# LI-Yiquan/3DPointCloudAttack

Measured on AMD Instinct MI355X. Metric: attack iters/s (B=32, N=1024, PointNet) + Chamfer HBM GB/s vs peak, higher is better.
Workload: dtype f32; 1 GPU; CW attack on PointNet(k=40, seeded random init), B=32 N=1024 fp32, UntargetedLogitsAdvLoss(kappa=30) + ChamferDist(adv2ori) + ClipPointsLinf(0.18), Adam lr 1e-2; one step = one hot-loop iteration for the whole batch; batch_per_gpu=32, points=1024, parallelism=independent attack instances x1

## Files before the change

3dpointcloudattack_amd/_lib.py:

```python
import ctypes
import os

import torch

from ctypes import c_char_p, c_float, c_int, c_int64, c_void_p

_HERE = os.path.dirname(os.path.abspath(__file__))
LIB_PATH = os.environ.get("PC3D_LIB_PATH") or os.path.join(_HERE, "libpc3d_hip.so")

_P = c_void_p
_I = c_int
_L = c_int64
_F = c_float
_D = ctypes.c_double
_PTS = [_P, _L, _L, _L]

SIGNATURES = {
    "pc3d_nn_f32": _PTS + _PTS + [_I, _I, _I, _P, _P, _P],
    "pc3d_nn_i64_f32": _PTS + _PTS + [_I, _I, _I, _P, _P, _P, _P],
    "pc3d_nn_bidir_f32": _PTS + _PTS + [_I, _I, _I, _P, _P, _P, _P, _P],
    "pc3d_nn_bidir_shared_ws_bytes": [_I, _I, _I],
    "pc3d_nn_bidir_shared_f32": _PTS + _PTS + [_I, _I, _I, _P, _P, _P, _P, _P, _L, _P],
    "pc3d_gemm_nt_f32": [_P, _L, _P, _P, _P, _L, _F, _I, _I, _I, _I, _F, _P, _L, _P],
    "pc3d_gemm_nt_tiled_f32": [_P, _L, _P, _P, _P, _L, _F, _I, _I, _I, _I, _F, _P, _L, _I, _P],
# ... 125 lines not shown
    "pc3d_pairwise_f32": _PTS + _PTS + [_I, _I, _I, _I, _P, _P],
    "pc3d_pointmlp3_tile_points": [],
    "pc3d_pointmlp3_max_fwd_f32": _PTS + [_I, _I] + [_P] * 7 + [_I, _I, _I, _I] + [_P] * 6 + [_P],
    "pc3d_pointmlp3_max_fwd_th_f32": _PTS + [_I, _I] + [_P, _P, _P, _I, _P] + [_P] * 6 + [_I, _I, _I, _I] + [_P] * 6 + [_P],
    "pc3d_pointmlp3_fold_f32": [_P, _P, _I, _I, _I, _I, _P, _P, _I, _P],
    "pc3d_pointmlp3_max_fwd_exact_f32": _PTS + [_I, _I] + [_P] * 7 + [_I, _I, _I, _I] + [_P] * 6 + [_P],
    "pc3d_pointmlp3_max_fwd_exact_th_f32": _PTS + [_I, _I] + [_P, _P, _P, _I, _P] + [_P] * 6 + [_I, _I, _I, _I] + [_P] * 6 + [_P],
    "pc3d_pointmlp3_max_fwd_screen_dbg_f32": _PTS + [_I, _I] + [_P, _P, _P, _P, _I, _P] + [_P] * 6 + [_I, _I, _I, _I]
    + [_P] * 6 + [_P, _P, _P, _I, _P],
    "pc3d_pointmlp3_w3_prepare_f32": [_P, _I, _P, _P, _P, _P],
    "pc3d_pointmlp3_max_fwd_prep_f32": _PTS + [_I, _I] + [_P] * 7 + [_I, _I, _I, _I] + [_P] * 6 + [_P, _P, _P] + [_P],
    "pc3d_pointmlp3_max_fwd_prep_th_f32": _PTS + [_I, _I] + [_P, _P, _P, _I, _P] + [_P] * 6 + [_I, _I, _I, _I] + [_P] * 6
    + [_P, _P, _P] + [_P],
    "pc3d_pointmlp3_max_fwd_screen_dbg_prep_f32": _PTS + [_I, _I] + [_P, _P, _P, _P, _I, _P] + [_P] * 6 + [_I, _I, _I, _I]
    + [_P] * 6 + [_P, _P, _P, _I] + [_P, _P, _P] + [_P],
    "pc3d_linear_pre_f32": [_P, _I, _I, _I, _P, _P, _I, _I, _I, _P, _I, _P, _I, _P, _I, _P],
    "pc3d_pointmlp3_max_bwd_f32": _PTS + [_I, _I] + [_P] * 7 + [_I, _I, _I] + [_P, _P, _P, _P] + _PTS + [_P, _I, _P],
    "pc3d_pointmlp3_max_bwd_twolist_f32": _PTS + [_I, _I] + [_P] * 7 + [_I, _I, _I] + [_P, _P, _P, _P] + _PTS + [_P, _I, _P],
    "pc3d_pointmlp3_max_bwd_tile32_f32": _PTS + [_I, _I] + [_P] * 7 + [_I, _I, _I] + [_P, _P, _P, _P] + _PTS + [_P, _I, _P],
    "pc3d_pointmlp3_max_bwd_packed_dbg_f32": _PTS + [_I, _I] + [_P] * 7 + [_I, _I, _I] + [_P, _P, _P, _P] + _PTS
    + [_P, _I, _I, _P],
    "pc3d_pointmlp3_bwd_tile_points": [],
    "pc3d_pointnet_ft_tower_fwd_f32": _PTS + [_I, _I] + [_P] * 6 + [_L] + [_P] * 3 + [_I] + [_P] * 5 + [_P],
    "pc3d_pointnet_ft_fold_w2_f32": [_P, _P, _I, _P, _P],
    "pc3d_pointnet_ft_tower_bwd_f32": _PTS + [_I, _I] + [_P] * 4 + [_L] + [_P, _P, _I] + [_P] * 5 + _PTS
    + [_P, _I, _I, _P, _I, _P],
    "pc3d_pointnet_ft_dtf_f32": _PTS + [_I, _I] + [_P] * 5 + [_P],
    "pc3d_linear_f32": [_P, _I, _I, _I, _I, _P, _P, _I, _I, _F, _P, _I, _F, _P, _I, _P],
    "pc3d_linear_nn_f32": [_P, _I, _I, _I, _I, _P, _P, _I, _I, _F, _P, _I, _F, _P, _I] + _PTS + _PTS
    + [_I, _I, _I, _P, _P, _I, _P],
# ... 77 lines not shown
```

3dpointcloudattack_amd/csrc/pointmlp.hip:

```cpp
#include <stdlib.h>
#include "pc3d_common.h"
#include "cw_update_body.h"
#include "pointmlp_body.h"

namespace pc3d {

__global__ __launch_bounds__(PM_FT) __attribute__((amdgpu_waves_per_eu(2, 2))) void pointmlp3_max_fwd_kernel(PMFwdArgs a) {
  __shared__ __attribute__((aligned(16))) float lds[PM_FWD_LDS_FLOATS];
  pm_fwd_prologue(a, lds);
  float* h2 = lds;
  const int tile = blockIdx.x, b = blockIdx.y;
  const int n0 = tile * PM_TP;
  const int lane = threadIdx.x & 63, wave = threadIdx.x >> 6;
  const int r = lane & 31, h = lane >> 5;

  const int ptile = wave & 3, cgrp = wave >> 2;
  float4 areg[PM_C2 / 8];
#pragma unroll
  for (int t = 0; t < PM_C2 / 8; ++t)
    areg[t] = *reinterpret_cast<const float4*>(h2 + (ptile * 32 + r) * PM_LD2 + 8 * t + 4 * h);
  __syncthreads();
  float* pv = lds;
  int* pi = reinterpret_cast<int*>(lds + 4 * PM_MAXC3F);
  const int nblk = a.C3 / 32;
// ... 1075 lines not shown
}

}

using namespace pc3d;

extern "C" int pc3d_pointmlp3_tile_points(void) { return PM_TP; }
extern "C" int pc3d_pointmlp3_bwd_tile_points(void) { return PM_BTP; }

static int pm_fwd_launch(const float* x, int64_t x_bs, int64_t x_ps, int64_t x_cs, int B, int N, const float* T,
                         const float* th_in, const float* th_W, const float* th_b, int th_K, float* th_out,
                         const float* W1, const float* b1, const float* W2, const float* b2, const float* W3,
                         const float* b3, int C1, int C2, int C3, int relu_last, float* part_val, int32_t* part_idx,
                         float* pooled, int32_t* argidx, uint64_t* mask1, uint32_t* mask2, void* stream,
                         bool exact = false, int32_t* stats = nullptr, float* dbg_S = nullptr, float* dbg_E = nullptr,
                         int stop_after = 0, const PMScreenPrep* prep = nullptr) {
  PC3D_REQUIRE(B >= 0 && N >= 1, "pc3d_pointmlp3_max_fwd_f32: bad sizes B=%d N=%d", B, N);
  PC3D_REQUIRE(C1 == PM_C1 && C2 == PM_C2 && C3 >= 32 && C3 % 32 == 0 && C3 <= PM_MAXC3F,
               "pc3d_pointmlp3_max_fwd_f32: unsupported widths %d/%d/%d (need 64/128/multiple of 32 <= 1024)", C1, C2, C3);
  PC3D_REQUIRE(B <= 65535, "pc3d_pointmlp3_max_fwd_f32: B=%d exceeds grid.y limit", B);
  if (B == 0) return PC3D_OK;
  PC3D_REQUIRE(x && W1 && b1 && W2 && b2 && W3 && b3 && part_val && part_idx,
               "pc3d_pointmlp3_max_fwd_f32: null pointer");
  PC3D_REQUIRE((pooled == nullptr) == (argidx == nullptr),
               "pc3d_pointmlp3_max_fwd_f32: pooled and argidx must both be given or both be NULL");
  PC3D_REQUIRE((mask1 == nullptr) == (mask2 == nullptr),
               "pc3d_pointmlp3_max_fwd_f32: mask1 and mask2 must both be given or both be NULL");
  const int ntiles = cdiv(N, PM_TP);
  PMFwdArgs a{{x, x_bs, x_ps, x_cs}, N, C3, ntiles, T, W1, b1, W2, b2, W3, b3, part_val, part_idx, mask1, mask2,
              th_in, th_W, th_b, th_K, th_out};
  hipStream_t st = as_stream(stream);
  int rc = 1;
  if (!exact) {
    rc = pm_fwd_screen_launch(a, B, stream, stats, dbg_S, dbg_E, stop_after, prep);
    if (rc < 0) return rc;
  }
  if (rc != 0) hipLaunchKernelGGL(pointmlp3_max_fwd_kernel, dim3(ntiles, B), dim3(PM_FT), 0, st, a);
  PC3D_LAUNCH_CHECK("pc3d_pointmlp3_max_fwd_f32");
  if (pooled) {
    hipLaunchKernelGGL(pointmlp3_fold_kernel<false>, dim3(cdiv(C3, 256), B), dim3(256), 0, st, part_val, part_idx, ntiles,
                       C3, relu_last, pooled, argidx);
    PC3D_LAUNCH_CHECK("pc3d_pointmlp3_max_fwd_f32/fold");
  }
  return PC3D_OK;
}

extern "C" int pc3d_pointmlp3_fold_f32(const float* part_val, const int32_t* part_idx, int B, int ntiles, int C3,
                                       int relu_last, float* pooled, int32_t* argidx, int serial, void* stream) {
  PC3D_REQUIRE(B >= 0 && B <= 65535 && ntiles >= 1 && C3 >= 1, "pc3d_pointmlp3_fold_f32: bad sizes B=%d ntiles=%d C3=%d", B,
// ... 122 lines not shown
                                                          const float* W3, const float* b3, int C1, int C2, int C3,
                                                          int relu_last, float* part_val, int32_t* part_idx, float* pooled,
                                                          int32_t* argidx, uint64_t* mask1, uint32_t* mask2, int32_t* stats,
                                                          float* dbg_S, float* dbg_E, int stop_after, const void* w3_bf,
                                                          const float* w3_nw, const float* w3_q, void* stream) {
  PC3D_REQUIRE(stats != nullptr, "pc3d_pointmlp3_max_fwd_screen_dbg_prep_f32: stats [B, ntiles, 2] is required");
  PC3D_REQUIRE((dbg_S == nullptr) == (dbg_E == nullptr), "pc3d_pointmlp3_max_fwd_screen_dbg_prep_f32: dbg_S and dbg_E go together");
  PC3D_REQUIRE(stop_after >= 0 && stop_after <= 3, "pc3d_pointmlp3_max_fwd_screen_dbg_prep_f32: stop_after = %d", stop_after);
  PC3D_REQUIRE(th_in == nullptr || (T == nullptr && th_W && th_b && T_out && th_K >= 1),
               "pc3d_pointmlp3_max_fwd_screen_dbg_prep_f32: T or a complete transform head, not both");
  PC3D_REQUIRE(w3_bf && w3_nw && w3_q, "pc3d_pointmlp3_max_fwd_screen_dbg_prep_f32: the prepared image needs w3_bf, w3_nw and w3_q");
  const PMScreenPrep q = pm_prep(w3_bf, w3_nw, w3_q);
  return pm_fwd_launch(x, x_bs, x_ps, x_cs, B, N, T, th_in, th_W, th_b, th_K, T_out, W1, b1, W2, b2, W3, b3, C1, C2, C3,
                       relu_last, part_val, part_idx, pooled, argidx, mask1, mask2, stream, false, stats, dbg_S, dbg_E,
                       stop_after, &q);
}

constexpr bool PM_BWD_DEFAULT_PACKED = true;
enum PMBwdForm { PM_BWD_PACKED = 0, PM_BWD_TILE32 = 1, PM_BWD_TWOLIST = 2 };

static int pm_bwd_launch(const char* who, int form, const float* x, int64_t x_bs, int64_t x_ps, int64_t x_cs, int B,
                         int N, const float* T, const float* W1, const float* b1, const float* W2, const float* b2,
                         const float* W3, const float* W2T, int C1, int C2, int C3, const int32_t* argidx,
                         const uint64_t* mask1, const uint32_t* mask2, const float* g_pooled, float* grad_x,
                         int64_t gx_bs, int64_t gx_ps, int64_t gx_cs, float* part_gT, int accumulate, void* stream) {
  PC3D_REQUIRE(B >= 0 && N >= 1, "%s: bad sizes B=%d N=%d", who, B, N);
  PC3D_REQUIRE(C1 == PM_C1 && C2 == PM_C2 && C3 >= 32 && C3 % 32 == 0 && C3 <= PM_MAXC3,
               "%s: unsupported widths %d/%d/%d", who, C1, C2, C3);
  PC3D_REQUIRE(B <= 65535, "%s: B=%d exceeds grid.y limit", who, B);
  if (B == 0) return PC3D_OK;
// ... 123 lines not shown
```

3dpointcloudattack_amd/csrc/pointmlp_body.h:

```cpp
#pragma once
#include "pc3d_common.h"

namespace pc3d {

using f32x16 = __attribute__((ext_vector_type(16))) float;

constexpr int PM_C1 = 64;
constexpr int PM_C2 = 128;
constexpr int PM_TP = 128;
constexpr int PM_LD1 = PM_C1 + 4;
constexpr int PM_LD2 = PM_C2 + 4;
constexpr int PM_BTP = 32;
constexpr int PM_MAXC3 = 1024;

__device__ __forceinline__ void load_point(const PtsView& x, const float* T, int b, int n, int N, float& px,
                                           float& py, float& pz) {
  px = py = pz = 0.f;
  if (n < N) {
    const float* p = x.p + (int64_t)b * x.bs + (int64_t)n * x.ps;
    const float x0 = p[0], x1 = p[x.cs], x2 = p[2 * x.cs];
    if (T) {
      const float* t = T;
      px = __builtin_fmaf(x2, t[6], __builtin_fmaf(x1, t[3], x0 * t[0]));
      py = __builtin_fmaf(x2, t[7], __builtin_fmaf(x1, t[4], x0 * t[1]));
// ... 139 lines not shown
      const int pt0 = n0 + (tl0 + tl) * 32 + (e & 3) + 8 * (e >> 2);
      uint32_t* m2 = a.mask2 + ((int64_t)b * a.N) * 4 + c2b;
      if (pt0 < a.N) m2[(int64_t)pt0 * 4] = (uint32_t)mine;
      if (pt0 + 4 < a.N) m2[(int64_t)(pt0 + 4) * 4] = (uint32_t)(mine >> 32);
    }
  }
  __syncthreads();
}


struct PMScreenPrep {
  const __attribute__((ext_vector_type(8))) __bf16* w3_bf;
  const float* w3_nw;
  const float4* w3_q;
};
int pm_fwd_screen_launch(const PMFwdArgs& a, int B, void* stream, int32_t* stats, float* dbg_S, float* dbg_E,
                         int stop_after, const PMScreenPrep* prep);
int pm_w3_prepare_launch(const float* W3, int C3, void* w3_bf, float* w3_nw, float* w3_q, void* stream);

}
```

3dpointcloudattack_amd/csrc/pointmlp_screen.hip:

```cpp
#include "pc3d_common.h"
#include "pointmlp_body.h"
#include "pointmlp_screen_bound.h"

namespace pc3d {

using bf16x8 = __attribute__((ext_vector_type(8))) __bf16;

constexpr int PMS_CAP = 128;
constexpr int PMS_SLOTS = PM_MAXC3F / 32 / (PM_FT / 64);
constexpr int PMS_WLIST = PMS_SLOTS * PMS_CAP;
constexpr int PMS_LDA = PM_C2 + 8;
constexpr size_t PMS_LDS_BYTES = (size_t)PM_FWD_LDS_FLOATS * 4 + PM_TP * 4 + (size_t)PM_MAXC3F * 8 +
                                 (PM_FT / 64) * PMS_WLIST * 2 + 2 * (size_t)PM_TP * PMS_LDA * 2;
static_assert(PMS_LDS_BYTES + 1024 <= 160 * 1024, "one workgroup's LDS on gfx950");
static_assert((PM_FWD_LDS_FLOATS * 4 + PM_TP * 4) % 8 == 0, "the keys are 8-byte aligned");
static_assert(PM_TP == 128 && PMS_SLOTS <= 4, "a list entry is slot << 12 | channel-in-block << 7 | point");

constexpr int PMS_PCAP = 8;
constexpr size_t PMS_A16_OFF = (size_t)PM_FWD_LDS_FLOATS * 4 + PM_TP * 4 + (size_t)PM_MAXC3F * 8 + (PM_FT / 64) * PMS_WLIST * 2;
constexpr size_t PMS_A16_OFF_PREP = (size_t)PM_FWD_LDS_FLOATS * 4 + PM_TP * 4 + (size_t)PM_MAXC3F * PMS_PCAP;
constexpr size_t PMS_LDS_BYTES_PREP = PMS_A16_OFF_PREP + 2 * (size_t)PM_TP * PMS_LDA * 2;
static_assert(PMS_LDS_BYTES_PREP <= PMS_LDS_BYTES && PMS_A16_OFF_PREP % 16 == 0 && PMS_A16_OFF % 16 == 0, "PREP's LDS map");
static_assert(PMS_PCAP >= 4 && PMS_PCAP <= 15, "a channel's candidate count is kept in 4 bits");

// ... 495 lines not shown
  }
  __builtin_amdgcn_fence(__ATOMIC_ACQ_REL, "wavefront");
  for (int i = lane; i < 32 * PMS_SLOTS; i += 64) {
    const int slot = i >> 5;
    if (!((screened >> slot) & 1u)) continue;
    const int c = (wave + (PM_FT / 64) * slot) * 32 + (i & 31);
    const unsigned long long key = s_key[c];
    const unsigned ord = (unsigned)(key >> 32), low = (unsigned)key;
    unsigned vb = (ord & 0x80000000u) ? (ord & 0x7fffffffu) : ~ord;
    if (low & 1u) vb = 0x80000000u;
    a.part_val[obase + c] = __builtin_bit_cast(float, vb) + a.b3[c];
    a.part_idx[obase + c] = n0 + 127 - (int)((low >> 1) & 127u);
  }
}

template <bool DBG, bool DUMP, bool PREP>
static int pms_launch_t(const PMFwdArgs& a, int B, hipStream_t st, const PMScreenDbg& d, const PMScreenPrep& q) {
  static bool done[64] = {};
  int dev = 0;
  PC3D_REQUIRE(hipGetDevice(&dev) == hipSuccess && dev >= 0 && dev < 64, "pointmlp3 screen: no current device");
  auto kernel = pointmlp3_max_fwd_screen_kernel<DBG, DUMP, PREP>;
  constexpr size_t lds = PREP ? PMS_LDS_BYTES_PREP : PMS_LDS_BYTES;
  if (!done[dev]) {
    hipStreamCaptureStatus cs = hipStreamCaptureStatusNone;
    if (hipStreamIsCapturing(st, &cs) != hipSuccess || cs != hipStreamCaptureStatusNone) {
      (void)hipGetLastError();
      return 1;
    }
    const hipError_t e = hipFuncSetAttribute(reinterpret_cast<const void*>(kernel),
                                             hipFuncAttributeMaxDynamicSharedMemorySize, (int)lds);
    PC3D_REQUIRE(e == hipSuccess, "pointmlp3 screen: hipFuncSetAttribute(MaxDynamicSharedMemorySize): %s", hipGetErrorString(e));
    done[dev] = true;
  }
  hipLaunchKernelGGL(kernel, dim3(a.ntiles, B), dim3(PM_FT), lds, st, a, d, q);
  return 0;
}

template <bool PREP>
static int pms_launch_form(const PMFwdArgs& a, int B, hipStream_t st, const PMScreenDbg& d, const PMScreenPrep& q) {
  if (d.dbg_S || d.dbg_E) return pms_launch_t<true, true, PREP>(a, B, st, d, q);
  if (d.stats || d.stop_after) return pms_launch_t<true, false, PREP>(a, B, st, d, q);
  return pms_launch_t<false, false, PREP>(a, B, st, d, q);
}

int pm_fwd_screen_launch(const PMFwdArgs& a, int B, void* stream, int32_t* stats, float* dbg_S, float* dbg_E,
                         int stop_after, const PMScreenPrep* prep) {
  const PMScreenDbg d{stats, dbg_S, dbg_E, stop_after};
  if (prep != nullptr && pms_launch_form<true>(a, B, as_stream(stream), d, *prep) == 0) return 0;
  return pms_launch_form<false>(a, B, as_stream(stream), d, PMScreenPrep{nullptr, nullptr, nullptr});
}

int pm_w3_prepare_launch(const float* W3, int C3, void* w3_bf, float* w3_nw, float* w3_q, void* stream) {
  hipLaunchKernelGGL(pms_w3_prepare_kernel, dim3(C3 / 32), dim3(64), 0, as_stream(stream), W3,
                     reinterpret_cast<bf16x8*>(w3_bf), w3_nw, reinterpret_cast<float4*>(w3_q), C3);
  return 0;
}

}
```

3dpointcloudattack_amd/ops.py:

```python
import contextlib
import os

import numpy as np
import torch

from . import _lib
from . import graphed as _graphed

DETERMINISTIC = os.environ.get("PC3D_DETERMINISTIC", "1") != "0"


def set_deterministic(on):
    global DETERMINISTIC
    was, DETERMINISTIC = DETERMINISTIC, bool(on)
    return was


@contextlib.contextmanager
def deterministic(on=True):
    was = set_deterministic(on)
    try:
        yield
    finally:
        set_deterministic(was)
# ... 296 lines not shown
    if part_idx.shape != part_val.shape or part_idx.dtype != torch.int32 or not (part_val.is_contiguous() and part_idx.is_contiguous()):
        raise ValueError("pointmlp3_fold_raw: part_val f32 / part_idx i32, both contiguous [B,ntiles,C3], expected")
    pooled = torch.empty((B, C3), dtype=torch.float32, device=part_val.device)
    argidx = torch.empty((B, C3), dtype=torch.int32, device=part_val.device)
    with torch.cuda.device(part_val.device):
        _lib.call("pc3d_pointmlp3_fold_f32", part_val.data_ptr(), part_idx.data_ptr(), B, ntiles, C3, 1 if relu_last else 0,
                  pooled.data_ptr(), argidx.data_ptr(), 1 if serial else 0, _stream())
    return pooled, argidx


def pointmlp3_w3_prepare(W3):
    _check(W3, "W3")
    C3 = W3.shape[0]
    if W3.dim() != 2 or W3.shape[1] != 128 or not W3.is_contiguous():
        raise ValueError("pointmlp3_w3_prepare: W3 must be a contiguous [C3,128] tensor")
    bf = torch.empty((C3 // 32, 8, 2, 64, 8), dtype=torch.bfloat16, device=W3.device)
    nw = torch.empty((C3,), dtype=torch.float32, device=W3.device)
    q = torch.empty((32, C3, 4), dtype=torch.float32, device=W3.device)
    with torch.cuda.device(W3.device):
        _lib.call("pc3d_pointmlp3_w3_prepare_f32", W3.data_ptr(), C3, bf.data_ptr(), nw.data_ptr(), q.data_ptr(), _stream())
    return bf, nw, q


def _pm_w3_pack(weights, W3):
    pack = weights[7] if len(weights) > 7 else None
    if not isinstance(pack, list):
        return None
    if not pack:
        if torch.cuda.is_current_stream_capturing():
            return None
        pack.extend(pointmlp3_w3_prepare(W3) + ((W3.data_ptr(), W3._version),))
    return pack[:3] if pack[3] == (W3.data_ptr(), W3._version) else None


def pointmlp3_max_fwd_raw(x, weights, relu_last, T=None, x_cf=True, fold=True, want_masks=False, T_head=None, serial=False,
                          exact=False, screen_dbg=None, in_launch=False):
    xp, xbs, xps, xcs, B, N = _pts(x, x_cf, "x")
    W1, b1, W2, b2, W3, b3 = weights[:6]
    for w in weights[:7]:
        _check(w, "weight")
        if not w.is_contiguous():
            raise ValueError("pointmlp3 weights must be contiguous")
    C1, C2, C3 = W1.shape[0], W2.shape[0], W3.shape[0]
    if T is not None:
        _check(T, "T")
        T = T.contiguous()
    ntiles = (N + _pm_tile() - 1) // _pm_tile()
    dev = x.device
    part_val = torch.empty((B, ntiles, C3), dtype=torch.float32, device=dev)
    part_idx = torch.empty((B, ntiles, C3), dtype=torch.int32, device=dev)
    pooled = torch.empty((B, C3), dtype=torch.float32, device=dev)
    argidx = torch.empty((B, C3), dtype=torch.int32, device=dev)
    masks = None
    if want_masks:
        masks = (torch.empty((B, N), dtype=torch.int64, device=dev), torch.empty((B, N, 4), dtype=torch.int32, device=dev))
    tail = (W1.data_ptr(), b1.data_ptr(), W2.data_ptr(), b2.data_ptr(), W3.data_ptr(), b3.data_ptr(),
            C1, C2, C3, 1 if relu_last else 0, part_val.data_ptr(), part_idx.data_ptr(),
            pooled.data_ptr() if fold and not serial else 0, argidx.data_ptr() if fold and not serial else 0,
            masks[0].data_ptr() if masks else 0, masks[1].data_ptr() if masks else 0, _stream())
    T_out = None
    if screen_dbg is not None and exact:
        raise ValueError("pointmlp3_max_fwd_raw: screen_dbg belongs to the screened launch, not to exact=True")
    sfx = "exact_" if exact else ""
    with torch.cuda.device(dev):
        prep = None if exact or in_launch else _pm_w3_pack(weights, W3)
        if prep is not None:
            sfx, prep = "prep_", tuple(t.data_ptr() for t in prep)
        if T_head is not None:
            if T is not None:
                raise ValueError("pointmlp3_max_fwd_raw: give T or T_head, not both")
            h, Wt, bt = T_head
            if h.shape[0] != B or Wt.shape != (9, h.shape[1]) or bt.numel() != 9 or not (h.is_contiguous() and Wt.is_contiguous()):
                raise ValueError("pointmlp3_max_fwd_raw: T_head = (h [B,K], W [9,K], b [9]) contiguous expected")
            T_out = torch.empty((B, 9), dtype=torch.float32, device=dev)
        if screen_dbg is not None:
            screen_dbg["stats"] = torch.zeros((B, ntiles, 2), dtype=torch.int32, device=dev)
            dS = dE = None
            if screen_dbg.get("dump"):
                dS = torch.full((B, N, C3), float("nan"), dtype=torch.float32, device=dev)
                dE = torch.full((B, N, C3), float("nan"), dtype=torch.float32, device=dev)
                screen_dbg["S"], screen_dbg["E"] = dS, dE
            th = (h.data_ptr(), Wt.data_ptr(), bt.data_ptr(), h.shape[1], T_out.data_ptr()) if T_head is not None else (0, 0, 0, 0, 0)
# ... 3255 lines not shown
```

include/pc3d.h:

```cpp
#ifndef PC3D_H
#define PC3D_H

#include <stdint.h>

#ifdef __cplusplus
extern "C" {
#endif

#define PC3D_OK 0
#define PC3D_EINVAL (-22)

int pc3d_version(void);
const char* pc3d_last_error(void);

int pc3d_nn_f32(const float* q, int64_t q_bs, int64_t q_ps, int64_t q_cs,
                const float* r, int64_t r_bs, int64_t r_ps, int64_t r_cs,
                int B, int N, int M, float* min_d2, int32_t* idx, void* stream);
int pc3d_nn_i64_f32(const float* q, int64_t q_bs, int64_t q_ps, int64_t q_cs,
                    const float* r, int64_t r_bs, int64_t r_ps, int64_t r_cs,
                    int B, int N, int M, float* min_d2, int32_t* idx, int64_t* idx64, void* stream);


int pc3d_nn_bidir_f32(const float* a, int64_t a_bs, int64_t a_ps, int64_t a_cs,
                      const float* b, int64_t b_bs, int64_t b_ps, int64_t b_cs,
// ... 149 lines not shown
int pc3d_pointmlp3_max_fwd_prep_th_f32(const float* x, int64_t x_bs, int64_t x_ps, int64_t x_cs, int B, int N,
                                       const float* th_in, const float* th_W, const float* th_b, int th_K, float* T_out,
                                       const float* W1, const float* b1, const float* W2, const float* b2,
                                       const float* W3, const float* b3, int C1, int C2, int C3, int relu_last,
                                       float* part_val, int32_t* part_idx, float* pooled, int32_t* argidx,
                                       uint64_t* mask1, uint32_t* mask2, const void* w3_bf, const float* w3_nw,
                                       const float* w3_q, void* stream);
int pc3d_pointmlp3_max_fwd_screen_dbg_prep_f32(const float* x, int64_t x_bs, int64_t x_ps, int64_t x_cs, int B, int N,
                                               const float* T, const float* th_in, const float* th_W, const float* th_b,
                                               int th_K, float* T_out, const float* W1, const float* b1, const float* W2,
                                               const float* b2, const float* W3, const float* b3, int C1, int C2, int C3,
                                               int relu_last, float* part_val, int32_t* part_idx, float* pooled,
                                               int32_t* argidx, uint64_t* mask1, uint32_t* mask2, int32_t* stats,
                                               float* dbg_S, float* dbg_E, int stop_after, const void* w3_bf,
                                               const float* w3_nw, const float* w3_q, void* stream);

int pc3d_pointmlp3_max_bwd_f32(const float* x, int64_t x_bs, int64_t x_ps, int64_t x_cs, int B, int N,
                               const float* T, const float* W1, const float* b1, const float* W2,
                               const float* b2, const float* W3, const float* W2T, int C1, int C2, int C3,
                               const int32_t* argidx, const uint64_t* mask1, const uint32_t* mask2,
                               const float* g_pooled,
                               float* grad_x, int64_t gx_bs, int64_t gx_ps, int64_t gx_cs,
                               float* part_gT, int accumulate, void* stream);
int pc3d_pointmlp3_max_bwd_twolist_f32(const float* x, int64_t x_bs, int64_t x_ps, int64_t x_cs, int B, int N,
                                       const float* T, const float* W1, const float* b1, const float* W2,
                                       const float* b2, const float* W3, const float* W2T, int C1, int C2, int C3,
                                       const int32_t* argidx, const uint64_t* mask1, const uint32_t* mask2,
                                       const float* g_pooled,
                                       float* grad_x, int64_t gx_bs, int64_t gx_ps, int64_t gx_cs,
                                       float* part_gT, int accumulate, void* stream);
// ... 451 lines not shown
```

Measured before the change: 5688 iters/s.

## Add fp16 screening path for the W3 max-pool forward with scaled weights

Adds an fp16 variant of the screened third-layer max-pool forward kernel. W3 is pre-scaled by a power of two into fp16 MFMA layout and activations are scaled per tile, which gives tighter error bounds than the existing bf16 screen. It uses 32x32x16 f16 MFMAs with per-channel candidate lists and falls back to exact recomputation when bounds fail. The prepared fp16 image sits in the same buffer as the bf16 image and is made the default form. This adds a prepare kernel and more LDS use, and risks more fallbacks if the scaling bounds are loose.

```diff
diff --git a/3dpointcloudattack_amd/_lib.py b/3dpointcloudattack_amd/_lib.py
--- a/3dpointcloudattack_amd/_lib.py
+++ b/3dpointcloudattack_amd/_lib.py
@@ -163,6 +163,12 @@
     + [_P, _P, _P] + [_P],
     "pc3d_pointmlp3_max_fwd_screen_dbg_prep_f32": _PTS + [_I, _I] + [_P, _P, _P, _P, _I, _P] + [_P] * 6 + [_I, _I, _I, _I]
     + [_P] * 6 + [_P, _P, _P, _I] + [_P, _P, _P] + [_P],
+    "pc3d_pointmlp3_w3_prepare_h_f32": [_P, _I, _P, _P, _P, _P],
+    "pc3d_pointmlp3_max_fwd_h_f32": _PTS + [_I, _I] + [_P] * 7 + [_I, _I, _I, _I] + [_P] * 6 + [_P] * 5 + [_P],
+    "pc3d_pointmlp3_max_fwd_h_th_f32": _PTS + [_I, _I] + [_P, _P, _P, _I, _P] + [_P] * 6 + [_I, _I, _I, _I] + [_P] * 6
+    + [_P] * 5 + [_P],
+    "pc3d_pointmlp3_max_fwd_screen_dbg_h_f32": _PTS + [_I, _I] + [_P, _P, _P, _P, _I, _P] + [_P] * 6 + [_I, _I, _I, _I]
+    + [_P] * 6 + [_P, _P, _P, _I] + [_P] * 5 + [_P],
     "pc3d_linear_pre_f32": [_P, _I, _I, _I, _P, _P, _I, _I, _I, _P, _I, _P, _I, _P, _I, _P],
     "pc3d_pointmlp3_max_bwd_f32": _PTS + [_I, _I] + [_P] * 7 + [_I, _I, _I] + [_P, _P, _P, _P] + _PTS + [_P, _I, _P],
     "pc3d_pointmlp3_max_bwd_twolist_f32": _PTS + [_I, _I] + [_P] * 7 + [_I, _I, _I] + [_P, _P, _P, _P] + _PTS + [_P, _I, _P],
diff --git a/3dpointcloudattack_amd/csrc/pointmlp.hip b/3dpointcloudattack_amd/csrc/pointmlp.hip
--- a/3dpointcloudattack_amd/csrc/pointmlp.hip
+++ b/3dpointcloudattack_amd/csrc/pointmlp.hip
@@ -1113,7 +1113,7 @@
                          const float* b3, int C1, int C2, int C3, int relu_last, float* part_val, int32_t* part_idx,
                          float* pooled, int32_t* argidx, uint64_t* mask1, uint32_t* mask2, void* stream,
                          bool exact = false, int32_t* stats = nullptr, float* dbg_S = nullptr, float* dbg_E = nullptr,
-                         int stop_after = 0, const PMScreenPrep* prep = nullptr) {
+                         int stop_after = 0, const PMScreenPrep* prep = nullptr, const PMScreenPrepH* hprep = nullptr) {
   PC3D_REQUIRE(B >= 0 && N >= 1, "pc3d_pointmlp3_max_fwd_f32: bad sizes B=%d N=%d", B, N);
   PC3D_REQUIRE(C1 == PM_C1 && C2 == PM_C2 && C3 >= 32 && C3 % 32 == 0 && C3 <= PM_MAXC3F,
                "pc3d_pointmlp3_max_fwd_f32: unsupported widths %d/%d/%d (need 64/128/multiple of 32 <= 1024)", C1, C2, C3);
@@ -1131,7 +1131,7 @@
   hipStream_t st = as_stream(stream);
   int rc = 1;
   if (!exact) {
-    rc = pm_fwd_screen_launch(a, B, stream, stats, dbg_S, dbg_E, stop_after, prep);
+    rc = pm_fwd_screen_launch(a, B, stream, stats, dbg_S, dbg_E, stop_after, prep, hprep);
     if (rc < 0) return rc;
   }
   if (rc != 0) hipLaunchKernelGGL(pointmlp3_max_fwd_kernel, dim3(ntiles, B), dim3(PM_FT), 0, st, a);
@@ -1284,6 +1284,75 @@
   return pm_fwd_launch(x, x_bs, x_ps, x_cs, B, N, T, th_in, th_W, th_b, th_K, T_out, W1, b1, W2, b2, W3, b3, C1, C2, C3,
                        relu_last, part_val, part_idx, pooled, argidx, mask1, mask2, stream, false, stats, dbg_S, dbg_E,
                        stop_after, &q);
+}
+
+extern "C" int pc3d_pointmlp3_w3_prepare_h_f32(const float* W3, int C3, const float* w3_nw, void* w3_h, float* w3_cw,
+                                               void* stream) {
+  PC3D_REQUIRE(C3 >= 32 && C3 % 32 == 0 && C3 <= PM_MAXC3F, "pc3d_pointmlp3_w3_prepare_h_f32: C3 = %d (need a multiple of 32 <= 1024)", C3);
+  PC3D_REQUIRE(W3 && w3_nw && w3_h && w3_cw, "pc3d_pointmlp3_w3_prepare_h_f32: null pointer");
+  pm_w3_prepare_h_launch(W3, C3, w3_nw, w3_h, w3_cw, stream);
+  PC3D_LAUNCH_CHECK("pc3d_pointmlp3_w3_prepare_h_f32");
+  return PC3D_OK;
+}
+
+static PMScreenPrepH pm_prep_h(const void* w3_h, const float* w3_cw, const float* w3_nw, const float* w3_q) {
+  return PMScreenPrepH{reinterpret_cast<decltype(PMScreenPrepH::w3_h)>(w3_h), w3_cw, w3_nw, reinterpret_cast<const float4*>(w3_q)};
+}
+
+extern "C" int pc3d_pointmlp3_max_fwd_h_f32(const float* x, int64_t x_bs, int64_t x_ps, int64_t x_cs, int B, int N,
+                                            const float* T, const float* W1, const float* b1, const float* W2,
+                                            const float* b2, const float* W3, const float* b3, int C1, int C2, int C3,
+                                            int relu_last, float* part_val, int32_t* part_idx, float* pooled,
+                                            int32_t* argidx, uint64_t* mask1, uint32_t* mask2, const void* w3_bf,
+                                            const float* w3_nw, const float* w3_q, const void* w3_h, const float* w3_cw,
+                                            void* stream) {
+  PC3D_REQUIRE(w3_bf && w3_nw && w3_q && w3_h && w3_cw, "pc3d_pointmlp3_max_fwd_h_f32: both prepared images are needed");
+  const PMScreenPrep q = pm_prep(w3_bf, w3_nw, w3_q);
+  const PMScreenPrepH qh = pm_prep_h(w3_h, w3_cw, w3_nw, w3_q);
+  return pm_fwd_launch(x, x_bs, x_ps, x_cs, B, N, T, nullptr, nullptr, nullptr, 0, nullptr, W1, b1, W2, b2, W3, b3, C1, C2,
+                       C3, relu_last, part_val, part_idx, pooled, argidx, mask1, mask2, stream, false, nullptr, nullptr,
+                       nullptr, 0, &q, &qh);
+}
+
+extern "C" int pc3d_pointmlp3_max_fwd_h_th_f32(const float* x, int64_t x_bs, int64_t x_ps, int64_t x_cs, int B, int N,
+                                               const float* th_in, const float* th_W, const float* th_b, int th_K,
+                                               float* T_out, const float* W1, const float* b1, const float* W2,
+                                               const float* b2, const float* W3, const float* b3, int C1, int C2, int C3,
+                                               int relu_last, float* part_val, int32_t* part_idx, float* pooled,
+                                               int32_t* argidx, uint64_t* mask1, uint32_t* mask2, const void* w3_bf,
+                                               const float* w3_nw, const float* w3_q, const void* w3_h,
+                                               const float* w3_cw, void* stream) {
+  PC3D_REQUIRE(th_in && th_W && th_b && T_out && th_K >= 1,
+               "pc3d_pointmlp3_max_fwd_h_th_f32: the transform head needs its input, weights [9,K], bias [9] and T_out");
+  PC3D_REQUIRE(w3_bf && w3_nw && w3_q && w3_h && w3_cw, "pc3d_pointmlp3_max_fwd_h_th_f32: both prepared images are needed");
+  const PMScreenPrep q = pm_prep(w3_bf, w3_nw, w3_q);
+  const PMScreenPrepH qh = pm_prep_h(w3_h, w3_cw, w3_nw, w3_q);
+  return pm_fwd_launch(x, x_bs, x_ps, x_cs, B, N, nullptr, th_in, th_W, th_b, th_K, T_out, W1, b1, W2, b2, W3, b3, C1, C2,
+                       C3, relu_last, part_val, part_idx, pooled, argidx, mask1, mask2, stream, false, nullptr, nullptr,
+                       nullptr, 0, &q, &qh);
+}
+
+extern "C" int pc3d_pointmlp3_max_fwd_screen_dbg_h_f32(const float* x, int64_t x_bs, int64_t x_ps, int64_t x_cs, int B,
+                                                       int N, const float* T, const float* th_in, const float* th_W,
+                                                       const float* th_b, int th_K, float* T_out, const float* W1,
+                                                       const float* b1, const float* W2, const float* b2, const float* W3,
+                                                       const float* b3, int C1, int C2, int C3, int relu_last,
+                                                       float* part_val, int32_t* part_idx, float* pooled, int32_t* argidx,
+                                                       uint64_t* mask1, uint32_t* mask2, int32_t* stats, float* dbg_S,
+                                                       float* dbg_E, int stop_after, const void* w3_bf, const float* w3_nw,
+                                                       const float* w3_q, const void* w3_h, const float* w3_cw,
+                                                       void* stream) {
+  PC3D_REQUIRE(stats != nullptr, "pc3d_pointmlp3_max_fwd_screen_dbg_h_f32: stats [B, ntiles, 2] is required");
+  PC3D_REQUIRE((dbg_S == nullptr) == (dbg_E == nullptr), "pc3d_pointmlp3_max_fwd_screen_dbg_h_f32: dbg_S and dbg_E go together");
+  PC3D_REQUIRE(stop_after >= 0 && stop_after <= 3, "pc3d_pointmlp3_max_fwd_screen_dbg_h_f32: stop_after = %d", stop_after);
+  PC3D_REQUIRE(th_in == nullptr || (T == nullptr && th_W && th_b && T_out && th_K >= 1),
+               "pc3d_pointmlp3_max_fwd_screen_dbg_h_f32: T or a complete transform head, not both");
+  PC3D_REQUIRE(w3_bf && w3_nw && w3_q && w3_h && w3_cw, "pc3d_pointmlp3_max_fwd_screen_dbg_h_f32: both prepared images are needed");
+  const PMScreenPrep q = pm_prep(w3_bf, w3_nw, w3_q);
+  const PMScreenPrepH qh = pm_prep_h(w3_h, w3_cw, w3_nw, w3_q);
+  return pm_fwd_launch(x, x_bs, x_ps, x_cs, B, N, T, th_in, th_W, th_b, th_K, T_out, W1, b1, W2, b2, W3, b3, C1, C2, C3,
+                       relu_last, part_val, part_idx, pooled, argidx, mask1, mask2, stream, false, stats, dbg_S, dbg_E,
+                       stop_after, &q, &qh);
 }
 
 constexpr bool PM_BWD_DEFAULT_PACKED = true;
diff --git a/3dpointcloudattack_amd/csrc/pointmlp_body.h b/3dpointcloudattack_amd/csrc/pointmlp_body.h
--- a/3dpointcloudattack_amd/csrc/pointmlp_body.h
+++ b/3dpointcloudattack_amd/csrc/pointmlp_body.h
@@ -177,8 +177,15 @@
   const float* w3_nw;
   const float4* w3_q;
 };
+struct PMScreenPrepH {
+  const __attribute__((ext_vector_type(8))) _Float16* w3_h;
+  const float* w3_cw;
+  const float* w3_nw;
+  const float4* w3_q;
+};
 int pm_fwd_screen_launch(const PMFwdArgs& a, int B, void* stream, int32_t* stats, float* dbg_S, float* dbg_E,
-                         int stop_after, const PMScreenPrep* prep);
+                         int stop_after, const PMScreenPrep* prep, const PMScreenPrepH* hprep = nullptr);
 int pm_w3_prepare_launch(const float* W3, int C3, void* w3_bf, float* w3_nw, float* w3_q, void* stream);
+int pm_w3_prepare_h_launch(const float* W3, int C3, const float* w3_nw, void* w3_h, float* w3_cw, void* stream);
 
 }
diff --git a/3dpointcloudattack_amd/csrc/pointmlp_screen.hip b/3dpointcloudattack_amd/csrc/pointmlp_screen.hip
--- a/3dpointcloudattack_amd/csrc/pointmlp_screen.hip
+++ b/3dpointcloudattack_amd/csrc/pointmlp_screen.hip
@@ -1,6 +1,7 @@
 #include "pc3d_common.h"
 #include "pointmlp_body.h"
 #include "pointmlp_screen_bound.h"
+#include "pointmlp_screen_h_bound.h"
 
 namespace pc3d {
 
@@ -533,6 +534,299 @@
   }
 }
 
+using f16x8 = __attribute__((ext_vector_type(8))) _Float16;
+
+constexpr int PMH_PCAP = 16;
+constexpr size_t PMH_AMAX_OFF = (size_t)PM_FWD_LDS_FLOATS * 4 + PM_TP * 4;
+constexpr size_t PMH_PTS_OFF = PMH_AMAX_OFF + 16;
+constexpr size_t PMH_A16_OFF = PMH_PTS_OFF + (size_t)PM_MAXC3F * PMH_PCAP;
+constexpr size_t PMH_LDS_BYTES = PMH_A16_OFF + (size_t)PM_TP * PMS_LDA * 2;
+static_assert(PMH_LDS_BYTES + 1024 <= 160 * 1024 && PMH_A16_OFF % 16 == 0 && PMH_PTS_OFF % 16 == 0, "H's LDS map");
+static_assert(PMH_PCAP >= 4 && PMH_PCAP <= 31 && 5 * PMS_SLOTS <= 32, "a channel's candidate count is kept in 5 bits per slot");
+static_assert(PM_TP <= 256, "a candidate point is one byte");
+
+__global__ __launch_bounds__(64) void pms_w3_prepare_h_kernel(const float* __restrict__ W3, const float* __restrict__ w3_nw,
+                                                              f16x8* __restrict__ w3_h, float* __restrict__ w3_cw) {
+  const int cb = blockIdx.x, lane = threadIdx.x;
+  const int r = lane & 31, h = lane >> 5;
+  const float nw = w3_nw[cb * 32 + r];
+  const bool ok = pms_norm_ok(nw);
+  const float two_sw = ok ? pmh_pow2(pmh_scale_exp(nw)) : 0.f;
+  const float* wrow = W3 + (int64_t)(cb * 32 + r) * PM_C2 + 8 * h;
+#pragma unroll
+  for (int t = 0; t < PM_C2 / 16; ++t) {
+    const float4 lo = *reinterpret_cast<const float4*>(wrow + 16 * t), hi = *reinterpret_cast<const float4*>(wrow + 16 * t + 4);
+    const float v[8] = {lo.x, lo.y, lo.z, lo.w, hi.x, hi.y, hi.z, hi.w};
+    f16x8 o;
+#pragma unroll
+    for (int i = 0; i < 8; ++i) o[i] = ok ? (_Float16)(v[i] * two_sw) : (_Float16)0.f;
+    w3_h[(cb * (PM_C2 / 16) + t) * 64 + lane] = o;
+  }
+  if (h == 0) w3_cw[cb * 32 + r] = ok ? pmh_cw(nw, two_sw) : __builtin_inff();
+}
+
+template <bool DBG, bool DUMP>
+__global__ __launch_bounds__(PM_FT) __attribute__((amdgpu_waves_per_eu(2, 2))) void pointmlp3_max_fwd_screen_h_kernel(
+    PMFwdArgs a, PMScreenDbg d, PMScreenPrepH w3) {
+  extern __shared__ __attribute__((aligned(16))) float pms_lds[];
+  float* h2 = pms_lds;
+  float* s_na = pms_lds + PM_FWD_LDS_FLOATS;
+  unsigned* s_amax = reinterpret_cast<unsigned*>(reinterpret_cast<char*>(pms_lds) + PMH_AMAX_OFF);
+  unsigned char* s_pts = reinterpret_cast<unsigned char*>(pms_lds) + PMH_PTS_OFF;
+  _Float16* s_a16 = reinterpret_cast<_Float16*>(reinterpret_cast<char*>(pms_lds) + PMH_A16_OFF);
+  const int tile = blockIdx.x, b = blockIdx.y;
+  const int n0 = tile * PM_TP;
+  const int nvalid = a.N - n0;
+  const int lane = threadIdx.x & 63, wave = threadIdx.x >> 6;
+  const int r = lane & 31, h = lane >> 5;
+  const int64_t obase = ((int64_t)b * a.ntiles + tile) * a.C3;
+  const int nblk = a.C3 / 32;
+  const int nslots = wave < nblk ? (nblk - wave + PM_FT / 64 - 1) / (PM_FT / 64) : 0;
+  const f16x8* wb = w3.w3_h + lane;
+  f16x8 q[PM_C2 / 16];
+  float cw_next = 0.f;
+  if (nslots > 0) {
+#pragma unroll
+    for (int t = 0; t < PM_C2 / 16; ++t) q[t] = wb[(wave * (PM_C2 / 16) + t) * 64];
+    cw_next = w3.w3_cw[wave * 32 + r];
+  }
+  if (threadIdx.x == 0) *s_amax = 0u;
+  pm_fwd_prologue(a, pms_lds);
+
+  bool bad;
+  float na;
+  float4 hv[8];
+  const int p = threadIdx.x >> 2, pq = threadIdx.x & 3;
+  {
+    const float* row = h2 + p * PM_LD2 + 32 * pq;
+    float ss = 0.f;
+#pragma unroll
+    for (int t = 0; t < 4; ++t) {
+      const float4 v = *reinterpret_cast<const float4*>(row + 8 * t), u = *reinterpret_cast<const float4*>(row + 8 * t + 4);
+      ss = __builtin_fmaf(v.x, v.x, ss), ss = __builtin_fmaf(v.y, v.y, ss);
+      ss = __builtin_fmaf(v.z, v.z, ss), ss = __builtin_fmaf(v.w, v.w, ss);
+      ss = __builtin_fmaf(u.x, u.x, ss), ss = __builtin_fmaf(u.y, u.y, ss);
+      ss = __builtin_fmaf(u.z, u.z, ss), ss = __builtin_fmaf(u.w, u.w, ss);
+      hv[2 * t] = v, hv[2 * t + 1] = u;
+    }
+    ss += __shfl_xor(ss, 1, 64);
+    ss += __shfl_xor(ss, 2, 64);
+    na = pms_norm_up(ss);
+    bad = !pms_norm_ok(na);
+    const float wmax = wave_max(na);
+    if (lane == 0) atomicMax(s_amax, __builtin_bit_cast(unsigned, wmax));
+  }
+  const bool tile_bad = __syncthreads_or(bad ? 1 : 0) != 0;
+  float two_sa = 1.f;
+  if (!tile_bad) {
+    const float amax = __builtin_bit_cast(float, *s_amax);
+    two_sa = pmh_pow2(pmh_scale_exp(amax));
+#pragma unroll
+    for (int t = 0; t < 4; ++t) {
+      const float4 v = hv[2 * t], u = hv[2 * t + 1];
+      const float x[8] = {v.x, v.y, v.z, v.w, u.x, u.y, u.z, u.w};
+      f16x8 o;
+#pragma unroll
+      for (int i = 0; i < 8; ++i) o[i] = (_Float16)(x[i] * two_sa);
+      *reinterpret_cast<f16x8*>(s_a16 + p * PMS_LDA + 32 * pq + 8 * t) = o;
+    }
+    if (pq == 0) s_na[p] = p < nvalid ? pmh_na(na, two_sa) : __builtin_inff();
+  }
+  __syncthreads();
+  if (DBG && d.stop_after == 1) return;
+
+  unsigned vmask[2] = {0u, 0u};
+#pragma unroll
+  for (int pt = 0; pt < 4; ++pt)
+#pragma unroll
+    for (int e = 0; e < 16; ++e) vmask[pt >> 1] |= (pms_point(pt, e, h) < nvalid) ? (1u << (16 * (pt & 1) + e)) : 0u;
+  unsigned screened = 0u, cnts = 0u;
+  int ncand = 0, nfall = 0;
+  float sink = 0.f;
+#pragma unroll 1
+  for (int slot = 0; slot < nslots; ++slot) {
+    const int cb = wave + (PM_FT / 64) * slot;
+    const int nxt = slot + 1 < nslots ? cb + PM_FT / 64 : cb;
+    const float cw = cw_next;
+    bool fall = tile_bad || __builtin_amdgcn_ballot_w64(!pmh_cw_ok(cw)) != 0ull;
+    if (!fall) {
+      f32x16 acc[4];
+#pragma unroll
+      for (int pt = 0; pt < 4; ++pt)
+#pragma unroll
+        for (int e = 0; e < 16; ++e) acc[pt][e] = 0.f;
+#pragma unroll
+      for (int t = 0; t < PM_C2 / 16; ++t) {
+        const f16x8 bq = q[t];
+        q[t] = wb[(nxt * (PM_C2 / 16) + t) * 64];
+#pragma unroll
+        for (int pt = 0; pt < 4; ++pt) {
+          const f16x8 ah = *reinterpret_cast<const f16x8*>(s_a16 + (pt * 32 + r) * PMS_LDA + 16 * t + 8 * h);
+          acc[pt] = __builtin_amdgcn_mfma_f32_32x32x16_f16(ah, bq, acc[pt], 0, 0, 0);
+        }
+      }
+      __builtin_amdgcn_sched_group_barrier(0x100, 2, 0);
+#pragma unroll
+      for (int g = 0; g < 4 * (PM_C2 / 16); ++g) {
+        if (g % 4 == 0) __builtin_amdgcn_sched_group_barrier(0x020, 1, 0);
+        __builtin_amdgcn_sched_group_barrier(0x008, 1, 0);
+        if (g + 2 < 4 * (PM_C2 / 16)) __builtin_amdgcn_sched_group_barrier(0x100, 1, 0);
+      }
+      __builtin_amdgcn_sched_group_barrier(0x020, 1, 0);
+      cw_next = w3.w3_cw[nxt * 32 + r];
+      if (DBG && d.stop_after == 2) {
+#pragma unroll
+        for (int pt = 0; pt < 4; ++pt)
+#pragma unroll
+          for (int e = 0; e < 16; ++e) sink += acc[pt][e];
+        continue;
+      }
+      if (DUMP && d.dbg_S != nullptr) {
+        int c3v = a.C3;
+        unsigned vm[2] = {vmask[0], vmask[1]};
+        asm volatile("" : "+v"(c3v), "+v"(vm[0]), "+v"(vm[1]));
+        const int64_t o0 = ((int64_t)b * a.N + n0) * a.C3 + cb * 32 + r;
+        const float back_a = 1.f / two_sa, back_w = 1.f / pmh_pow2(pmh_scale_exp(w3.w3_nw[cb * 32 + r]));
+#pragma unroll
+        for (int pt = 0; pt < 4; ++pt)
+#pragma unroll
+          for (int e = 0; e < 16; ++e) {
+            const int pp = pms_point(pt, e, h);
+            if ((vm[pt >> 1] >> (16 * (pt & 1) + e)) & 1u) {
+              d.dbg_S[o0 + (int64_t)pp * c3v] = acc[pt][e] * back_a * back_w;
+              d.dbg_E[o0 + (int64_t)pp * c3v] = pms_E(s_na[pp], cw) * back_a * back_w;
+            }
+          }
+      }
+      unsigned flags[2];
+      float L = pms_lower(acc, s_na, cw, h);
+      L = fmaxf(L, __shfl_xor(L, 32, 64));
+      pms_flags(acc, s_na, cw, h, L, flags);
+      flags[0] &= vmask[0], flags[1] &= vmask[1];
+      const int cnt = __builtin_popcount(flags[0]) + __builtin_popcount(flags[1]);
+      const int other = __shfl_xor(cnt, 32, 64);
+      if (__builtin_amdgcn_ballot_w64(cnt + other > PMH_PCAP) != 0ull) {
+        fall = true;
+      } else {
+        unsigned char* mine = s_pts + (cb * 32 + r) * PMH_PCAP + (h ? other : 0);
+#pragma unroll
+        for (int wd = 0; wd < 2; ++wd) {
+          unsigned f = flags[wd];
+          while (f) {
+            const int bit = __builtin_ctz(f);
+            f &= f - 1;
+            *mine++ = (unsigned char)pms_point(2 * wd + (bit >> 4), bit & 15, h);
+          }
+        }
+        cnts |= (unsigned)(cnt + other) << (5 * slot);
+        screened |= 1u << slot;
+        if (DBG) ncand += h ? 0 : cnt + other;
+      }
+    } else {
+#pragma unroll
+      for (int t = 0; t < PM_C2 / 16; ++t) q[t] = wb[(nxt * (PM_C2 / 16) + t) * 64];
+      cw_next = w3.w3_cw[nxt * 32 + r];
+    }
+    if (fall) {
+      pms_exact_block(h2, a.W3, a.b3, cb, n0, a.N, a.part_val + obase, a.part_idx + obase);
+      ++nfall;
+    }
+  }
+  if (DBG && d.stop_after == 2) {
+    if (sink == 12345.678f) a.part_val[obase] = sink;
+    return;
+  }
+  if (DBG && d.stats != nullptr) {
+    ncand = wave_sum(ncand);
+    if (lane == 0) {
+      int32_t* st = d.stats + ((int64_t)b * a.ntiles + tile) * 2;
+      if (ncand) atomicAdd(st, ncand);
+      if (nfall) atomicAdd(st + 1, nfall);
+    }
+  }
+  if (DBG && d.stop_after == 3) {
+    if (cnts == 0xffffffffu) a.part_val[obase] = 0.f;
+    return;
+  }
+
+  __builtin_amdgcn_fence(__ATOMIC_ACQ_REL, "wavefront");
+#pragma unroll 1
+  for (int j = 0; 2 * j < nslots; ++j) {
+    const int sl = 2 * j + h;
+    const bool live = sl < nslots && ((screened >> sl) & 1u);
+    const int n = live ? (int)((cnts >> (5 * sl)) & 31u) : 0;
+    if (__builtin_amdgcn_ballot_w64(n > 0) == 0ull) continue;
+    const int c = (wave + (PM_FT / 64) * (live ? sl : 0)) * 32 + r;
+    float4 wv[PM_C2 / 4];
+#pragma unroll
+    for (int t = 0; t < PM_C2 / 4; ++t) wv[t] = w3.w3_q[(int64_t)t * a.C3 + c];
+    unsigned long long key = 0ull;
+#pragma unroll 1
+    for (int i = 0; i < PMH_PCAP; ++i) {
+      if (__builtin_amdgcn_ballot_w64(i < n) == 0ull) break;
+      const int pc = i < n ? s_pts[c * PMH_PCAP + i] : 0;
+      const float4* ar = reinterpret_cast<const float4*>(h2 + pc * PM_LD2);
+      __builtin_amdgcn_sched_barrier(0);
+      float v = 0.f;
+#pragma unroll
+      for (int t = 0; t < PM_C2 / 8; ++t) {
+        const float4 a0 = ar[2 * t], a1 = ar[2 * t + 1];
+        const float4 w0 = wv[2 * t], w1 = wv[2 * t + 1];
+        v = __builtin_fmaf(a0.x, w0.x, v), v = __builtin_fmaf(a1.x, w1.x, v);
+        v = __builtin_fmaf(a0.y, w0.y, v), v = __builtin_fmaf(a1.y, w1.y, v);
+        v = __builtin_fmaf(a0.z, w0.z, v), v = __builtin_fmaf(a1.z, w1.z, v);
+        v = __builtin_fmaf(a0.w, w0.w, v), v = __builtin_fmaf(a1.w, w1.w, v);
+      }
+      __builtin_amdgcn_sched_group_barrier(0x100, 8, 0);
+#pragma unroll
+      for (int g = 0; g < PM_C2 / 8; ++g) {
+        __builtin_amdgcn_sched_group_barrier(0x002, 8, 0);
+        if (g + 4 < PM_C2 / 8) __builtin_amdgcn_sched_group_barrier(0x100, 2, 0);
+      }
+      const unsigned vb = __builtin_bit_cast(unsigned, v);
+      const unsigned zb = (v == 0.f) ? 0u : vb;
+      const unsigned ord = (zb & 0x80000000u) ? ~zb : (zb | 0x80000000u);
+      const unsigned low = ((unsigned)(127 - pc) << 1) | ((vb == 0x80000000u) ? 1u : 0u);
+      const unsigned long long k = ((unsigned long long)ord << 32) | low;
+      if (i < n && k > key) key = k;
+    }
+    if (live) {
+      const unsigned ord = (unsigned)(key >> 32), low = (unsigned)key;
+      unsigned vb = (ord & 0x80000000u) ? (ord & 0x7fffffffu) : ~ord;
+      if (low & 1u) vb = 0x80000000u;
+      a.part_val[obase + c] = __builtin_bit_cast(float, vb) + a.b3[c];
+      a.part_idx[obase + c] = n0 + 127 - (int)((low >> 1) & 127u);
+    }
+  }
+}
+
+template <bool DBG, bool DUMP>
+static int pms_launch_h_t(const PMFwdArgs& a, int B, hipStream_t st, const PMScreenDbg& d, const PMScreenPrepH& q) {
+  static bool done[64] = {};
+  int dev = 0;
+  PC3D_REQUIRE(hipGetDevice(&dev) == hipSuccess && dev >= 0 && dev < 64, "pointmlp3 screen: no current device");
+  auto kernel = pointmlp3_max_fwd_screen_h_kernel<DBG, DUMP>;
+  if (!done[dev]) {
+    hipStreamCaptureStatus cs = hipStreamCaptureStatusNone;
+    if (hipStreamIsCapturing(st, &cs) != hipSuccess || cs != hipStreamCaptureStatusNone) {
+      (void)hipGetLastError();
+      return 1;
+    }
+    const hipError_t e = hipFuncSetAttribute(reinterpret_cast<const void*>(kernel),
+                                             hipFuncAttributeMaxDynamicSharedMemorySize, (int)PMH_LDS_BYTES);
+    PC3D_REQUIRE(e == hipSuccess, "pointmlp3 screen: hipFuncSetAttribute(MaxDynamicSharedMemorySize): %s", hipGetErrorString(e));
+    done[dev] = true;
+  }
+  hipLaunchKernelGGL(kernel, dim3(a.ntiles, B), dim3(PM_FT), PMH_LDS_BYTES, st, a, d, q);
+  return 0;
+}
+
+static int pms_launch_h(const PMFwdArgs& a, int B, hipStream_t st, const PMScreenDbg& d, const PMScreenPrepH& q) {
+  if (d.dbg_S || d.dbg_E) return pms_launch_h_t<true, true>(a, B, st, d, q);
+  if (d.stats || d.stop_after) return pms_launch_h_t<true, false>(a, B, st, d, q);
+  return pms_launch_h_t<false, false>(a, B, st, d, q);
+}
+
 template <bool DBG, bool DUMP, bool PREP>
 static int pms_launch_t(const PMFwdArgs& a, int B, hipStream_t st, const PMScreenDbg& d, const PMScreenPrep& q) {
   static bool done[64] = {};
@@ -563,8 +857,9 @@
 }
 
 int pm_fwd_screen_launch(const PMFwdArgs& a, int B, void* stream, int32_t* stats, float* dbg_S, float* dbg_E,
-                         int stop_after, const PMScreenPrep* prep) {
+                         int stop_after, const PMScreenPrep* prep, const PMScreenPrepH* hprep) {
   const PMScreenDbg d{stats, dbg_S, dbg_E, stop_after};
+  if (hprep != nullptr && pms_launch_h(a, B, as_stream(stream), d, *hprep) == 0) return 0;
   if (prep != nullptr && pms_launch_form<true>(a, B, as_stream(stream), d, *prep) == 0) return 0;
   return pms_launch_form<false>(a, B, as_stream(stream), d, PMScreenPrep{nullptr, nullptr, nullptr});
 }
@@ -575,4 +870,10 @@
   return 0;
 }
 
-}
+int pm_w3_prepare_h_launch(const float* W3, int C3, const float* w3_nw, void* w3_h, float* w3_cw, void* stream) {
+  hipLaunchKernelGGL(pms_w3_prepare_h_kernel, dim3(C3 / 32), dim3(64), 0, as_stream(stream), W3, w3_nw,
+                     reinterpret_cast<f16x8*>(w3_h), w3_cw);
+  return 0;
+}
+
+}
diff --git a/3dpointcloudattack_amd/csrc/pointmlp_screen_h_bound.h b/3dpointcloudattack_amd/csrc/pointmlp_screen_h_bound.h
--- /dev/null
+++ b/3dpointcloudattack_amd/csrc/pointmlp_screen_h_bound.h
@@ -0,0 +1,17 @@
+#pragma once
+#include "pointmlp_screen_bound.h"
+
+namespace pc3d {
+
+constexpr float PMH_C = 0x1.1p-10f;
+constexpr float PMH_NA_FLOOR = 1.0f;
+constexpr int PMH_EXP = 13;
+constexpr float PMH_CW_MAX = 0x1p5f;
+
+PMS_HD inline int pmh_scale_exp(float n) { return PMH_EXP + 127 - (int)((__builtin_bit_cast(unsigned, n) >> 23) & 0xffu); }
+PMS_HD inline float pmh_pow2(int s) { return __builtin_bit_cast(float, (unsigned)(s + 127) << 23); }
+PMS_HD inline float pmh_na(float na, float two_sa) { return na * two_sa + PMH_NA_FLOOR; }
+PMS_HD inline float pmh_cw(float nw, float two_sw) { return PMH_C * (nw * two_sw); }
+PMS_HD inline bool pmh_cw_ok(float cw) { return cw < PMH_CW_MAX; }
+
+}
diff --git a/3dpointcloudattack_amd/ops.py b/3dpointcloudattack_amd/ops.py
--- a/3dpointcloudattack_amd/ops.py
+++ b/3dpointcloudattack_amd/ops.py
@@ -334,12 +334,29 @@
     C3 = W3.shape[0]
     if W3.dim() != 2 or W3.shape[1] != 128 or not W3.is_contiguous():
         raise ValueError("pointmlp3_w3_prepare: W3 must be a contiguous [C3,128] tensor")
-    bf = torch.empty((C3 // 32, 8, 2, 64, 8), dtype=torch.bfloat16, device=W3.device)
+    buf = torch.empty((C3 * _PM_W3_BYTES,), dtype=torch.uint8, device=W3.device)
+    bf = buf[:C3 * 512].view(torch.bfloat16).view(C3 // 32, 8, 2, 64, 8)
     nw = torch.empty((C3,), dtype=torch.float32, device=W3.device)
     q = torch.empty((32, C3, 4), dtype=torch.float32, device=W3.device)
     with torch.cuda.device(W3.device):
         _lib.call("pc3d_pointmlp3_w3_prepare_f32", W3.data_ptr(), C3, bf.data_ptr(), nw.data_ptr(), q.data_ptr(), _stream())
+        _lib.call("pc3d_pointmlp3_w3_prepare_h_f32", W3.data_ptr(), C3, nw.data_ptr(), bf.data_ptr() + C3 * 512,
+                  bf.data_ptr() + C3 * 768, _stream())
     return bf, nw, q
+
+
+_PM_W3_BYTES = 512 + 256 + 4
+
+
+def _pm_w3_h(bf):
+    C3 = bf.shape[0] * 32
+    st = bf.untyped_storage()
+    if bf.storage_offset() != 0 or st.nbytes() < C3 * _PM_W3_BYTES:
+        return None
+    raw = torch.empty(0, dtype=torch.uint8, device=bf.device).set_(st, 0, (C3 * _PM_W3_BYTES,))
+    h = raw[C3 * 512:C3 * 768].view(torch.float16).view(C3 // 32, 8, 64, 8)
+    cw = raw[C3 * 768:].view(torch.float32)
+    return (h, cw), (bf.data_ptr() + C3 * 512, bf.data_ptr() + C3 * 768)
 
 
 def _pm_w3_pack(weights, W3):
@@ -353,8 +370,11 @@
     return pack[:3] if pack[3] == (W3.data_ptr(), W3._version) else None
 
 
+PM_FWD_DEFAULT_FORM = "fp16"
+
+
 def pointmlp3_max_fwd_raw(x, weights, relu_last, T=None, x_cf=True, fold=True, want_masks=False, T_head=None, serial=False,
-                          exact=False, screen_dbg=None, in_launch=False):
+                          exact=False, screen_dbg=None, in_launch=False, form=None):
     xp, xbs, xps, xcs, B, N = _pts(x, x_cf, "x")
     W1, b1, W2, b2, W3, b3 = weights[:6]
     for w in weights[:7]:
@@ -384,8 +404,15 @@
     sfx = "exact_" if exact else ""
     with torch.cuda.device(dev):
         prep = None if exact or in_launch else _pm_w3_pack(weights, W3)
+        if form not in (None, "bf16", "fp16"):
+            raise ValueError("pointmlp3_max_fwd_raw: form is None, 'bf16' or 'fp16'")
+        if form is None:
+            form = PM_FWD_DEFAULT_FORM if screen_dbg is None else "bf16"
         if prep is not None:
+            hp = _pm_w3_h(prep[0]) if form == "fp16" else None
             sfx, prep = "prep_", tuple(t.data_ptr() for t in prep)
+            if hp is not None:
+                sfx, prep = "h_", prep + hp[1]
         if T_head is not None:
             if T is not None:
                 raise ValueError("pointmlp3_max_fwd_raw: give T or T_head, not both")
diff --git a/include/pc3d.h b/include/pc3d.h
--- a/include/pc3d.h
+++ b/include/pc3d.h
@@ -187,6 +187,29 @@
                                                int32_t* argidx, uint64_t* mask1, uint32_t* mask2, int32_t* stats,
                                                float* dbg_S, float* dbg_E, int stop_after, const void* w3_bf,
                                                const float* w3_nw, const float* w3_q, void* stream);
+int pc3d_pointmlp3_w3_prepare_h_f32(const float* W3, int C3, const float* w3_nw, void* w3_h, float* w3_cw, void* stream);
+int pc3d_pointmlp3_max_fwd_h_f32(const float* x, int64_t x_bs, int64_t x_ps, int64_t x_cs, int B, int N, const float* T,
+                                 const float* W1, const float* b1, const float* W2, const float* b2, const float* W3,
+                                 const float* b3, int C1, int C2, int C3, int relu_last, float* part_val,
+                                 int32_t* part_idx, float* pooled, int32_t* argidx, uint64_t* mask1, uint32_t* mask2,
+                                 const void* w3_bf, const float* w3_nw, const float* w3_q, const void* w3_h,
+                                 const float* w3_cw, void* stream);
+int pc3d_pointmlp3_max_fwd_h_th_f32(const float* x, int64_t x_bs, int64_t x_ps, int64_t x_cs, int B, int N,
+                                    const float* th_in, const float* th_W, const float* th_b, int th_K, float* T_out,
+                                    const float* W1, const float* b1, const float* W2, const float* b2,
+                                    const float* W3, const float* b3, int C1, int C2, int C3, int relu_last,
+                                    float* part_val, int32_t* part_idx, float* pooled, int32_t* argidx,
+                                    uint64_t* mask1, uint32_t* mask2, const void* w3_bf, const float* w3_nw,
+                                    const float* w3_q, const void* w3_h, const float* w3_cw, void* stream);
+int pc3d_pointmlp3_max_fwd_screen_dbg_h_f32(const float* x, int64_t x_bs, int64_t x_ps, int64_t x_cs, int B, int N,
+                                            const float* T, const float* th_in, const float* th_W, const float* th_b,
+                                            int th_K, float* T_out, const float* W1, const float* b1, const float* W2,
+                                            const float* b2, const float* W3, const float* b3, int C1, int C2, int C3,
+                                            int relu_last, float* part_val, int32_t* part_idx, float* pooled,
+                                            int32_t* argidx, uint64_t* mask1, uint32_t* mask2, int32_t* stats,
+                                            float* dbg_S, float* dbg_E, int stop_after, const void* w3_bf,
+                                            const float* w3_nw, const float* w3_q, const void* w3_h, const float* w3_cw,
+                                            void* stream);
 
 int pc3d_pointmlp3_max_bwd_f32(const float* x, int64_t x_bs, int64_t x_ps, int64_t x_cs, int B, int N,
                                const float* T, const float* W1, const float* b1, const float* W2,
```

Measured after the change: 6029 iters/s, median of 6. 6.0% higher.
